# worldbench/lidarcrafter

Hardware: AMD Instinct MI355X
Metric: denoising-steps/sec, nuScenes 32×1024 range image, 1/2/4/8 GPU (higher is better)
Workload: dtype f16x2-split MFMA, fp32 accumulate (fp32-class accuracy)

## Files before the change

lidarcrafter_amd/csrc/conv_f16x2.hip:

```cpp
#include "conv_f16x2_common.h"

using namespace lcconv;

namespace {

#if LC_TIMING
__device__ unsigned long long lc_dbg[32];
#endif

#ifndef LC_NP_AUX
#define LC_NP_AUX LC_DEF_AUX
#endif
template <class C, bool WIDE = false, bool EMIT = false>
__global__ __launch_bounds__(256, (C::BN > 64 && C::NTAP == 9) ? 1 : 2) void conv_f16x2_kernel(ConvArgsH a) {
    constexpr int HALO = C::HALO, NTAP = C::NTAP, BN = C::BN;
    constexpr int XR = C::XR, XW = C::XW;
    constexpr int KS = 2 * HALO + 1;
    constexpr int CB = (NTAP == 1 && WIDE) ? ((BN <= 64 && C::TH_ * C::TW_ <= 128) ? 8 : 4) : C::CB;
    constexpr int XU = CB * XR * XW, NXU = (XU + 255) / 256;
    constexpr int WU = NTAP * CB * BN, NWU = (WU + 255) / 256;
    __shared__ half8 lds[2 * XU + 2 * WU];
    __shared__ f32x4 ctab[GN_MAX_C];
    __shared__ float2 gtab[GN_MAX_G];
    half8* xh = lds;
// ... 330 lines not shown
                        : OOB_W;
    }
    const unsigned w_chunk = (unsigned)CB * (unsigned)a.Cop * 16u;
    auto dma_w = [&](half8* buf, int q, int ch) {
        if (!(LC_ABLATE & 2)) lds_dma16(rs_w, (lds_vptr)(buf + loff_w[q]), voff_w[q], (unsigned)ch * w_chunk);
    };

    auto load_x = [&](float (&xr)[NXU][8], int ch) {
#pragma unroll
        for (int i = 0; i < NXU; ++i)
#pragma unroll
            for (int k = 0; k < 8; ++k)
                xr[i][k] = __builtin_bit_cast(
                    float, __builtin_amdgcn_raw_buffer_load_b32(rsrc, x_voff[i],
                                                                (unsigned)(ch * 16 + k) * HW * 4u, 0));
    };

    for (int i = tid; i < BN; i += NT)
        bias_s[i] = (a.bias && co0 + i < a.Co) ? a.bias[co0 + i] * (1.0f / out_unscale) : 0.0f;
    const int kh = lane >> 5, l31 = lane & 31;
    f32x16 acc[C::TCO_][C::TPX_];
    auto acc_init = [&]() {
#pragma unroll
        for (int i = 0; i < C::TCO_; ++i)
#pragma unroll
            for (int m = 0; m < 4; ++m) {
                const f32x4 bq = *reinterpret_cast<const f32x4*>(&bias_s[(wco * C::TCO_ + i) * 32 + 8 * m + 4 * kh]);
#pragma unroll
                for (int j = 0; j < C::TPX_; ++j) {
                    acc[i][j][4 * m] = bq.x; acc[i][j][4 * m + 1] = bq.y;
                    acc[i][j][4 * m + 2] = bq.z; acc[i][j][4 * m + 3] = bq.w;
                }
            }
    };

    int xbase[C::TPX_];
#pragma unroll
    for (int j = 0; j < C::TPX_; ++j) {
        const int t = wpx * C::TPX_ + j;
        const int tr = t / C::TPR, tc = t - tr * C::TPR;
        xbase[j] = kh * (XR * XW) + tr * XW + tc * 32 + l31;
    }
    const int wbase = kh * BN + wco * C::TCO_ * 32 + l31;

    const float silu_c = -1.4426950408889634f * a.range->x_unscale;
    half8 st_hi[NXU], st_lo[NXU];
    auto read_row = [&](int i, int q, int ch) -> f32x4 {
        if constexpr (GNM != 0) {
            const f32x4* g = x_ok[i] ? ctab + ch * 8 + x_cb[i] * 4 : ctab + (a.Cgn >> 1);
            return g[q];
        } else {
            return f32x4{0.f, 0.f, 0.f, 0.f};
        }
    };
    auto stage_pair = [&](float (&xr)[NXU][8], int i, int q, const f32x4 row) {
        if (LC_ABLATE & 1) { asm volatile("" ::"v"(xr[i][2 * q]), "v"(xr[i][2 * q + 1])); return; }
        half2v ph, pl;
        if constexpr (GNM != 0) {
            f32x2 v = {xr[i][2 * q], xr[i][2 * q + 1]};
            const f32x2 A = {row.x, row.y}, Bv = {row.z, row.w};
            v = __builtin_elementwise_fma(v, A, Bv);
            if constexpr (GNM == 1) {
                const f32x2 t = v * silu_c;
                f32x2 e = {__builtin_amdgcn_exp2f(t.x), __builtin_amdgcn_exp2f(t.y)};
                e = e + 1.0f;
                const f32x2 rc = {__builtin_amdgcn_rcpf(e.x), __builtin_amdgcn_rcpf(e.y)};
                v = v * rc;
            }
            pair_split_amax(v.x, v.y, ph, pl, am);
        } else {
            pair_split_scale<false>(xr[i][2 * q], xr[i][2 * q + 1], xs, ph, pl, am);
        }
        st_hi[i][2 * q] = ph.x; st_hi[i][2 * q + 1] = ph.y;
        st_lo[i][2 * q] = pl.x; st_lo[i][2 * q + 1] = pl.y;
    };
    auto commit_x = [&](half8* buf, int i) {
        if (LC_ABLATE & 1) return;
        const int d = x_rc[i] >= 0 ? x_cb[i] * PL + ((x_rc[i] >> 16) & 0xFFF) * XW + (x_rc[i] & 0xFFFF) : XU;
        buf[d] = st_hi[i];
        buf[XUP + d] = st_lo[i];
    };
    constexpr int NSTEP = 4 * NXU;
    constexpr int SPT = NTAP == 1 ? NSTEP : ((NSTEP + NTAP - 2) / (NTAP - 1) > 2 ? (NSTEP + NTAP - 2) / (NTAP - 1) : 2);
    auto step_tap = [](int st) {
        if (NTAP == 1) return 0;
        const int ntaps = (NSTEP + SPT - 1) / SPT;
        const int first = NTAP - 1 - ntaps > 0 ? NTAP - 1 - ntaps : 0;
        return first + st / SPT;
    };
    typedef DefEpi<C, EMIT_STATS> DE;
    DE de;
    auto compute = [&](const half8* cur, half8* nxt, float (&xr)[NXU][8], int chn, int dslot0) {
        const half8* cxh = cur;
        const half8* cxl = cur + XUP;
        const half8* cwh = cur + 2 * XUP;
        const half8* cwl = cwh + WS;
        half8 ah[2][C::TCO_], al[2][C::TCO_], bh[2][C::TPX_], bl[2][C::TPX_];
        auto fetch = [&](int tap, int s) {
            const int dy = tap / KS, dx = tap - dy * KS;
#pragma unroll
            for (int i = 0; i < C::TCO_; ++i) {
                ah[s][i] = cwh[tap * CB * BN + wbase + i * 32];
                al[s][i] = cwl[tap * CB * BN + wbase + i * 32];
            }
#pragma unroll
            for (int j = 0; j < C::TPX_; ++j) {
                bh[s][j] = cxh[xbase[j] + dy * XW + dx];
                bl[s][j] = cxl[xbase[j] + dy * XW + dx];
            }
        };
        fetch(0, 0);
#if LC_DMA_FIRST
        if (NTAP != 1) {
#pragma unroll
            for (int q = 0; q < KW; ++q) dma_w(nxt, q, chn);
        }
#endif
#pragma unroll
        for (int tap = 0; tap < NTAP; ++tap) {
            const int s = (LC_ABLATE & 4) ? 0 : (tap & 1);
            f32x4 rows[SPT];
            if (LC_PIPE_ROWS && GNM != 0) {
#pragma unroll
                for (int st = 0; st < NSTEP; ++st)
                    if (tap == step_tap(st)) rows[st % SPT] = read_row(st >> 2, st & 3, chn);
                __builtin_amdgcn_sched_barrier(0);
            }
            if (tap + 1 < NTAP && !(LC_ABLATE & 4)) fetch(tap + 1, s ^ 1);
            __builtin_amdgcn_sched_barrier(0);
            if (dslot0 >= 0 && dslot0 + tap < DE::NUSED) de.slot(dslot0 + tap);
            if (NTAP == 1) {
#pragma unroll
                for (int q = 0; q < KW; ++q) dma_w(nxt, q, chn);
            } else if (tap < KW && !LC_DMA_FIRST) {
                dma_w(nxt, tap, chn);
            }
#pragma unroll
            for (int st = 0; st < NSTEP; ++st)
                if (tap == step_tap(st)) {
                    stage_pair(xr, st >> 2, st & 3,
                               (LC_PIPE_ROWS && GNM != 0) ? rows[st % SPT] : read_row(st >> 2, st & 3, chn));
                    if ((st & 3) == 3) commit_x(nxt, st >> 2);
                }
            if (LC_ABLATE & 32) {
#pragma unroll
                for (int i = 0; i < C::TCO_; ++i) asm volatile("" ::"v"(ah[s][i]), "v"(al[s][i]));
#pragma unroll
                for (int j = 0; j < C::TPX_; ++j) asm volatile("" ::"v"(bh[s][j]), "v"(bl[s][j]));
                __builtin_amdgcn_sched_barrier(0);
                continue;
            }
            if (LC_F16X2_TERMS & 2) {
#pragma unroll
                for (int i = 0; i < C::TCO_; ++i)
#pragma unroll
                    for (int j = 0; j < C::TPX_; ++j)
                        acc[i][j] = __builtin_amdgcn_mfma_f32_32x32x16_f16(al[s][i], bh[s][j], acc[i][j], 0, 0, 0);
            }
            if (LC_F16X2_TERMS & 4) {
#pragma unroll
                for (int i = 0; i < C::TCO_; ++i)
#pragma unroll
                    for (int j = 0; j < C::TPX_; ++j)
                        acc[i][j] = __builtin_amdgcn_mfma_f32_32x32x16_f16(ah[s][i], bl[s][j], acc[i][j], 0, 0, 0);
            }
#pragma unroll
            for (int i = 0; i < C::TCO_; ++i)
#pragma unroll
                for (int j = 0; j < C::TPX_; ++j)
                    acc[i][j] = __builtin_amdgcn_mfma_f32_32x32x16_f16(ah[s][i], bh[s][j], acc[i][j], 0, 0, 0);
            __builtin_amdgcn_sched_barrier(0);
        }
    };

    half8* cur = lds;
    half8* nxt = lds + BUF;
    const int nchunk = a.Cib / CB;
    const int last = nchunk - 1;
    float xr[NXU][8];
    load_x(xr, 0);
#pragma unroll
    for (int q = 0; q < KW; ++q) dma_w(cur, q, 0);
    if constexpr (GNM != 0) {
        if (a.gs.partials) {
            for (int i = tid; i < a.Cgn; i += NT) ctab[i] = gn_row_from_stats(a.gs, xb, b, i, a.Ci, HW);
        } else if (a.segs.seg[0].p) {
            gn_rows_from_ostats<NT>(a, b, tid, ctab, gtab);
        } else {
            const f32x4* g = a.gn + (long long)b * a.Cgn;
            for (int i = tid; i < a.Cgn; i += NT) ctab[i] = g[i];
        }
        __syncthreads();
        constexpr int NQ = (GN_MAX_C / 2 + NT - 1) / NT;
        const int npair = a.Cgn >> 1;
        f32x4 qd[NQ];
#pragma unroll
        for (int k = 0; k < NQ; ++k) {
            const int p = tid + k * NT;
            if (p < npair) {
                const f32x4 r0 = ctab[2 * p], r1 = ctab[2 * p + 1];
                qd[k] = f32x4{r0.y * xs, r1.y * xs, fmaf(-r0.x, r0.y, r0.z) * xs, fmaf(-r1.x, r1.y, r1.z) * xs};
            }
        }
        __syncthreads();
#pragma unroll
        for (int k = 0; k < NQ; ++k) {
            const int p = tid + k * NT;
            if (p < npair) ctab[p] = qd[k];
        }
        if (tid < 4) ctab[npair + tid] = f32x4{0.f, 0.f, 0.f, 0.f};
        __syncthreads();
    }
#pragma unroll
    for (int i = 0; i < NXU; ++i) {
#pragma unroll
        for (int q = 0; q < 4; ++q) stage_pair(xr, i, q, read_row(i, q, 0));
        commit_x(cur, i);
    }
    asm volatile("s_waitcnt vmcnt(0)" ::: "memory");
    __syncthreads();
    const int co_wave = co0 + wco * C::TCO_ * 32 + 4 * kh;
    float* yb = a.y + (long long)b * a.y_bs;
    const float* rb = (a.res && !(LC_ABLATE & 16)) ? a.res + (long long)b * a.res_bs : nullptr;
    de.init(yb, rb, a.Co, HW, out_unscale, a.out_scale, co_wave,
            a.ostats ? a.ostats + (long long)b * (a.Co >> (a.ounit == 2 ? 1 : 3)) * a.oslots : nullptr, a.oslots,
            a.ounit);
    acc_init();
#if LC_TIMING
    unsigned long long t_comp = 0, t_bar = 0, t_epi = 0, n_chunk = 0;
    const unsigned long long t_start = __builtin_amdgcn_s_memtime();
#endif
    auto k_iter = [&](int nxt_ch, int dslot0) {
        if (!(LC_ABLATE & 2)) load_x(xr, nxt_ch);
        __builtin_amdgcn_sched_barrier(0);
#if LC_TIMING
        const unsigned long long ta = __builtin_amdgcn_s_memtime();
#endif
        compute(cur, nxt, xr, nxt_ch, dslot0);
#if LC_TIMING
        const unsigned long long tb = __builtin_amdgcn_s_memtime();
#endif
        {
            int later = 0;
#pragma unroll
            for (int tap = (NTAP == 1 ? 1 : (LC_DMA_FIRST ? 0 : KW)); tap < NTAP; ++tap) {
                const int sl = dslot0 + tap;
                if (dslot0 >= 0 && sl < DE::NUSED) later += DE::ops_of(sl);
            }
            wait_vmcnt(later);
        }
        asm volatile("s_waitcnt lgkmcnt(0)" ::: "memory");
        __builtin_amdgcn_s_barrier();
        asm volatile("" ::: "memory");
#if LC_TIMING
        t_comp += tb - ta; t_bar += __builtin_amdgcn_s_memtime() - tb; ++n_chunk;
#endif
        half8* t = cur; cur = nxt; nxt = t;
    };
    for (int tile = 0; tile < tpb; ++tile) {
        const bool more = tile + 1 < tpb;
        auto iter = [&](int ch, int dslot0) {
            if (ch == last && more) set_tile(h0 + dh, w0 + dw);
            k_iter(ch == last ? (more ? 0 : last) : ch + 1, dslot0);
        };
#pragma unroll
        for (int c = 0; c < DE::DCH; ++c)
            if (c < nchunk) iter(c, c * NTAP);
        if (nchunk < DE::DCH) {
            if (nchunk == 1) de.flush_from(NTAP);
            else if (nchunk == 2) de.flush_from(2 * NTAP);
            else de.flush_from(3 * NTAP);
        }
        for (int ch = DE::DCH; ch < nchunk; ++ch) iter(ch, -1);
        de.begin(acc, h0, w0, H, W, wpx, lane, a.tiles_w, HW, co0 + wco * C::TCO_ * 32, more);
        if (more) acc_init();
        h0 += dh; w0 += dw;
    }
#if LC_TIMING
    const unsigned long long te0 = __builtin_amdgcn_s_memtime();
#endif
    de.drain(acc);
#if LC_TIMING
    t_epi = __builtin_amdgcn_s_memtime() - te0;
#endif
    publish_amax(a.range, am, amax_seen);
#if LC_TIMING
    if (lane == 0) {
        atomicAdd(&lc_dbg[0], __builtin_amdgcn_s_memtime() - t_start);
        atomicAdd(&lc_dbg[1], t_start - t_enter);
        atomicAdd(&lc_dbg[2], t_comp);
        atomicAdd(&lc_dbg[3], t_bar);
        atomicAdd(&lc_dbg[4], t_epi);
        atomicAdd(&lc_dbg[5], n_chunk);
        atomicAdd(&lc_dbg[6], 1ull);
    }
#endif
}


#include "conv_f16x2_pp.h"

#include "conv_f16x2_ps.h"

template <class C>
int launch_pipe(ConvArgsH a, hipStream_t st) {
    a.tiles_h = (a.H + C::TH_ - 1) / C::TH_;
    a.tiles_w = (a.W + C::TW_ - 1) / C::TW_;
    const int ncot = (a.Co + C::BN - 1) / C::BN;
    const long long n_tiles = (long long)a.B * a.tiles_h * a.tiles_w * ncot;
    auto max_tpb = [&](int extent) {
        int t = 1;
        while (t < 4 && extent % (t * 2) == 0 && n_tiles / (t * 2) >= 256) t *= 2;
        return t;
    };
    static const int vert_env = [] { const char* e = getenv("LC_CONV_VERT"); return e ? atoi(e) : 1; }();
    static const int xcd_env = [] { const char* e = getenv("LC_CONV_XCD"); return e ? atoi(e) : 1; }();
    const int tpb_h = max_tpb(a.tiles_h), tpb_w = max_tpb(a.tiles_w);
    int vert = vert_env && tpb_h >= tpb_w;
    int tpb = vert ? tpb_h : tpb_w;
    if (C::NTAP == 1) tpb = 1;
    if (a.tpb > 0) {
        tpb = a.tpb;
        vert = vert_env && a.tiles_h % tpb == 0;
        if (!vert && a.tiles_w % tpb) tpb = 1;
    }
    if (a.part) tpb = 1;
    a.tpb = tpb;
    a.vert = vert;
    dim3 grid(a.B * a.tiles_h * a.tiles_w / tpb, ncot);
    a.xcd = (xcd_env && grid.x % 8 == 0 && grid.x >= 16) ? 1 : 0;

    if (a.xsp) {
        if constexpr (C::NTAP == 9) {
            if (a.part) grid.z = a.ksplit;
            if (a.ostats && !a.part) hipLaunchKernelGGL((conv_f16x2_ps_kernel<C, true>), grid, dim3(C::NT), 0, st, a);
            else hipLaunchKernelGGL((conv_f16x2_ps_kernel<C, false>), grid, dim3(C::NT), 0, st, a);
            return lc_launch_status();
        } else {
            return LC_EUNSUP;
        }
    }
    {
        const long long d = (const char*)a.wl - (const char*)a.wh;
        if (d <= 0 || d >= (1ll << 31)) return LC_EINVAL;
        if (d + (long long)C::NTAP * a.Cib * a.Cop * 16 >= (1ll << 31)) return LC_EUNSUP;
    }
    const int gnm = a.gn ? (a.gn_silu ? 1 : 2) : 0;
#define LC_PIPE_LAUNCH(E, G) hipLaunchKernelGGL((conv_f16x2_pipe_kernel<C, E, G>), grid, dim3(C::NT), 0, st, a)
    if (a.ostats && a.ounit == 2) {
        if constexpr (C::NTAP == 9) {
            if (gnm == 1) LC_PIPE_LAUNCH(2, 1); else if (gnm == 2) LC_PIPE_LAUNCH(2, 2); else LC_PIPE_LAUNCH(2, 0);
        } else {
            return LC_EUNSUP;
        }
    } else if (a.ostats) {
        if (gnm == 1) LC_PIPE_LAUNCH(1, 1); else if (gnm == 2) LC_PIPE_LAUNCH(1, 2); else LC_PIPE_LAUNCH(1, 0);
    } else {
        if (gnm == 1) LC_PIPE_LAUNCH(0, 1); else if (gnm == 2) LC_PIPE_LAUNCH(0, 2); else LC_PIPE_LAUNCH(0, 0);
    }
#undef LC_PIPE_LAUNCH
    return lc_launch_status();
}

template <class C>
int launch_h(ConvArgsH a, hipStream_t st) {
    a.tiles_h = (a.H + C::TH_ - 1) / C::TH_;
    a.tiles_w = (a.W + C::TW_ - 1) / C::TW_;
    dim3 grid(a.B * a.tiles_h * a.tiles_w, (a.Co + C::BN - 1) / C::BN);
    if constexpr (C::NTAP == 1) {
        const bool wide = (long long)grid.x * grid.y <= 512;
        if (a.ostats) {
            if (a.ounit != 8) return LC_EUNSUP;
            if (wide) hipLaunchKernelGGL((conv_f16x2_kernel<C, true, true>), grid, dim3(256), 0, st, a);
            else hipLaunchKernelGGL((conv_f16x2_kernel<C, false, true>), grid, dim3(256), 0, st, a);
            return lc_launch_status();
        }
        if (wide) {
            hipLaunchKernelGGL((conv_f16x2_kernel<C, true>), grid, dim3(256), 0, st, a);
            return lc_launch_status();
        }
    } else if (a.ostats) {
        return LC_EUNSUP;
    }
    hipLaunchKernelGGL((conv_f16x2_kernel<C, false>), grid, dim3(256), 0, st, a);
    return lc_launch_status();
}

bool pp_eligible(int Ci, int Co, int H, int W, int ks) {
    return ks == 3 && Ci % 16 == 0 && Ci >= 64 && Ci <= PPG::MAX_C && Co % 64 == 0 && H % 4 == 0 && W % 64 == 0;
}
int launch_pp(ConvArgsH a, hipStream_t st) {
    if (!pp_eligible(a.Ci, a.Co, a.H, a.W, 3) || a.xsp || a.part) return LC_EUNSUP;
    if (a.gn && a.Cgn > PPG::MAX_C) return LC_EUNSUP;
    a.tiles_h = a.H / PPG::TH;
    a.tiles_w = a.W / PPG::TW;
    const int ncot = a.Co / PPG::BN;
    const long long strips = (long long)a.B * a.tiles_h * a.tiles_w * ncot;
    int ns = 1;
    while (ns < 8 && a.tiles_h % (2 * ns) == 0 && strips / (2 * ns) >= 256) ns *= 2;
    if (a.tpb > 0 && a.tiles_h % a.tpb == 0) ns = a.tpb;
    a.tpb = ns;
    dim3 grid(a.B * a.tiles_h * a.tiles_w / ns, ncot);
    static const int xcd_env = [] { const char* e = getenv("LC_CONV_XCD"); return e ? atoi(e) : 1; }();
    a.xcd = (xcd_env && grid.x % 8 == 0 && grid.x >= 16) ? 1 : 0;
    a.vert = 1;
    {
        const long long d = (const char*)a.wl - (const char*)a.wh;
        if (d <= 0 || d >= (1ll << 31)) return LC_EINVAL;
        if (d + (long long)PPG::NTAP * a.Cib * a.Cop * 16 >= (1ll << 31)) return LC_EUNSUP;
    }
    const int gnm = a.gn ? (a.gn_silu ? 1 : 2) : 0;
#define LC_PP_LAUNCH(E, G) hipLaunchKernelGGL((conv_f16x2_pp_kernel<E, G>), grid, dim3(PPG::NT), 0, st, a)
    if (a.ostats && a.ounit == 2) {
        if (gnm == 1) LC_PP_LAUNCH(2, 1); else if (gnm == 2) LC_PP_LAUNCH(2, 2); else LC_PP_LAUNCH(2, 0);
    } else if (a.ostats) {
        if (gnm == 1) LC_PP_LAUNCH(1, 1); else if (gnm == 2) LC_PP_LAUNCH(1, 2); else LC_PP_LAUNCH(1, 0);
    } else {
        if (gnm == 1) LC_PP_LAUNCH(0, 1); else if (gnm == 2) LC_PP_LAUNCH(0, 2); else LC_PP_LAUNCH(0, 0);
    }
#undef LC_PP_LAUNCH
    return lc_launch_status();
}

template <int KS>
int dispatch_h(int cfg, const ConvArgsH& a, hipStream_t st) {
    switch (cfg) {
        case 1: return launch_h<HCfg<2, 2, 2, 2, 2, 64, KS>>(a, st);
        case 2: return launch_h<HCfg<1, 4, 2, 2, 4, 64, KS>>(a, st);
        case 3: return launch_h<HCfg<2, 2, 1, 1, 2, 32, KS>>(a, st);
        case 4: return launch_h<HCfg<2, 2, 2, 2, 4, 32, KS>>(a, st);
        case 5: return launch_h<HCfg<1, 4, 2, 1, 2, 64, KS>>(a, st);
        case 12: return launch_pipe<HCfg<1, 4, 2, 2, 4, 64, KS>>(a, st);
        case 13: return launch_pipe<HCfg<2, 2, 1, 1, 2, 32, KS>>(a, st);
        case 15: return launch_pipe<HCfg<1, 4, 2, 1, 2, 64, KS>>(a, st);
        case 22: return launch_pipe<HCfg<1, 8, 2, 1, 4, 64, KS>>(a, st);
        case 23: return launch_pipe<HCfg<2, 4, 1, 2, 4, 64, KS>>(a, st);
        case 25: return launch_pipe<HCfg<2, 4, 1, 1, 2, 64, KS>>(a, st);
        case 27:
            if (KS == 3 && tall_eligible(a)) return launch_tall(a, st);
            return launch_pipe<HCfg<2, 4, 1, 2, 4, 64, KS>>(a, st);
        case 28: return launch_pipe<HCfg<1, 8, 1, 1, 4, 64, KS>>(a, st);
        case 33: return KS == 3 ? launch_pp(a, st) : LC_EUNSUP;
        default: return LC_EUNSUP;
    }
}

int pipe_stat_slots(int cfg, int H, int W, int ks = 3) {
    int th, tw, wpx;
    switch (cfg) {
        case 1: if (ks != 1) return 0; th = 2; tw = 64; wpx = 2; break;
        case 2: if (ks != 1) return 0; th = 4; tw = 64; wpx = 4; break;
        case 3: if (ks != 1) return 0; th = 2; tw = 32; wpx = 2; break;
        case 4: if (ks != 1) return 0; th = 4; tw = 32; wpx = 2; break;
        case 5: if (ks != 1) return 0; th = 2; tw = 64; wpx = 4; break;
        case 12: th = 4; tw = 64; wpx = 4; break;
        case 13: th = 2; tw = 32; wpx = 2; break;
        case 15: th = 2; tw = 64; wpx = 4; break;
        case 22: th = 4; tw = 64; wpx = 8; break;
        case 23: th = 4; tw = 64; wpx = 4; break;
        case 25: th = 2; tw = 64; wpx = 4; break;
        case 27: th = 4; tw = 64; wpx = 4; break;
        case 28: th = 4; tw = 64; wpx = 8; break;
        case 33: th = 4; tw = 64; wpx = 4; break;
        default: return 0;
    }
    return ((H + th - 1) / th) * ((W + tw - 1) / tw) * wpx;
}

int auto_cfg_h(int B, int Ci, int Co, int H, int W, int ks) {
    const long long px = (long long)B * H * W;
    auto blocks = [&](int bn, int pxb) { return ((Co + bn - 1) / bn) * ((px + pxb - 1) / pxb); };
    const bool t256 = H % 4 == 0 && W % 64 == 0, t128 = H % 2 == 0 && W % 64 == 0;
    if (ks == 1) {
        if (t256 && blocks(64, 256) > 192 && blocks(64, 256) <= 256) return 23;
        return (t128 && blocks(64, 128) >= 512) ? 5 : 3;
    }
    if (Ci >= 24) {
        if (Co <= 32 && t256 && blocks(64, 256) >= 256) return 28;
        static const long long pp_min = [] { const char* e = getenv("LC_PP_MIN_STRIPS"); return e ? atoll(e) : 0ll; }();
        if (pp_min > 0 && pp_eligible(Ci, Co, H, W, ks) && blocks(64, 256) >= pp_min) return 33;
        if (t256 && blocks(64, 256) >= 256) {
            static const int tall_env = [] { const char* e = getenv("LC_TALL"); return e ? atoi(e) : 1; }();
            if (tall_env && ks == 3 && (Ci == 32 || Ci == 64)) return 27;
            return 23;
        }
        if (t128 && blocks(64, 128) >= 256) return 25;
        return 13;
    }
    if (t256 && blocks(64, 256) >= 256 && Ci >= 64) return 2;
    if (t128 && blocks(64, 128) >= 512) return 5;
    return 3;
}

__global__ void weight_amax_kernel(const float* __restrict__ w, long long n, float* wmeta) {
    float am = 0.0f;
    for (long long e = blockIdx.x * (long long)blockDim.x + threadIdx.x; e < n;
         e += (long long)gridDim.x * blockDim.x)
        am = fmaxf(am, fabsf(w[e]));
    lc_block_amax_publish(am, reinterpret_cast<unsigned*>(wmeta + 2));
}

__device__ __forceinline__ float weight_scale_for(float amax) {
    if (!(amax > 0.0f) || !(amax < 3.0e38f)) return W_PRESCALE_DEFAULT;
    const float A = amax * W_PRESCALE_DEFAULT;
    if (A >= 32.0f && A <= 32768.0f) return W_PRESCALE_DEFAULT;
    int e;
    frexpf(amax, &e);
    int k = 13 - e;
    k = k < -120 ? -120 : (k > 120 ? 120 : k);
    return ldexpf(1.0f, k);
}

template <bool DX>
__device__ __forceinline__ void pack_weight_elems(const float* __restrict__ w, _Float16* __restrict__ ph,
                                                  _Float16* __restrict__ pl, int Co, int Ci, int ntap, int Cib,
                                                  int Cop, float ws, long long first, long long stride) {
    const long long n = (long long)ntap * Cib * Cop * 8;
    for (long long e = first; e < n; e += stride) {
        const int k = e & 7;
        long long r = e >> 3;
        const int co = r % Cop; r /= Cop;
        const int cb = r % Cib;
        const int tap = r / Cib;
        const int ci = cb * 8 + k;
        float v = 0.0f;
        if (co < Co && ci < Ci)
            v = (DX ? w[((long long)ci * Co + co) * ntap + (ntap - 1 - tap)]
                    : w[((long long)co * Ci + ci) * ntap + tap]) * ws;
        _Float16 hf, lf;
        f16x2_split_scalar(v, hf, lf);
        ph[e] = hf;
        pl[e] = lf;
    }
}

template <bool DX>
__global__ void pack_weight_h_kernel(const float* __restrict__ w, _Float16* __restrict__ ph,
                                     _Float16* __restrict__ pl, int Co, int Ci, int ntap, int Cib,
                                     int Cop, float* wmeta, const float* __restrict__ amax_src) {
    const float amax = amax_src ? amax_src[2] : wmeta[2];
    const float ws = weight_scale_for(amax);
    if (blockIdx.x == 0 && threadIdx.x == 0) {
        wmeta[0] = ws; wmeta[1] = 1.0f / ws;
        if (amax_src) { wmeta[2] = amax; wmeta[3] = 0.0f; }
    }
    pack_weight_elems<DX>(w, ph, pl, Co, Ci, ntap, Cib, Cop, ws, blockIdx.x * (long long)blockDim.x + threadIdx.x,
                          (long long)gridDim.x * blockDim.x);
}

__global__ void multi_weight_zero_kernel(const lc_weight_pack_job* __restrict__ jobs, int n) {
    const int j = blockIdx.x * blockDim.x + threadIdx.x;
    if (j < n) jobs[j].fwd_meta[2] = 0.0f;
}
__global__ void multi_weight_amax_kernel(const lc_weight_pack_job* __restrict__ jobs) {
    const lc_weight_pack_job jb = jobs[blockIdx.y];
    const long long n = (long long)jb.Co * jb.Ci * jb.ks * jb.ks;
    float am = 0.0f;
    for (long long e = blockIdx.x * (long long)blockDim.x + threadIdx.x; e < n; e += (long long)gridDim.x * blockDim.x)
        am = fmaxf(am, fabsf(jb.w[e]));
    lc_block_amax_publish(am, reinterpret_cast<unsigned*>(jb.fwd_meta + 2));
}
__global__ void multi_weight_pack_kernel(const lc_weight_pack_job* __restrict__ jobs) {
    const lc_weight_pack_job jb = jobs[blockIdx.y];
    const float amax = jb.fwd_meta[2];
    const float ws = weight_scale_for(amax);
    const int ntap = jb.ks * jb.ks;
    const long long first = blockIdx.x * (long long)blockDim.x + threadIdx.x, stride = (long long)gridDim.x * blockDim.x;
    if (blockIdx.z == 0) {
        if (blockIdx.x == 0 && threadIdx.x == 0) { jb.fwd_meta[0] = ws; jb.fwd_meta[1] = 1.0f / ws; }
        pack_weight_elems<false>(jb.w, (_Float16*)jb.fwd_hi, (_Float16*)jb.fwd_lo, jb.Co, jb.Ci, ntap,
                                 (jb.Ci + 15) / 16 * 2, (jb.Co + 63) / 64 * 64, ws, first, stride);
    } else {
        if (blockIdx.x == 0 && threadIdx.x == 0) {
            jb.dx_meta[0] = ws; jb.dx_meta[1] = 1.0f / ws; jb.dx_meta[2] = amax; jb.dx_meta[3] = 0.0f;
        }
        pack_weight_elems<true>(jb.w, (_Float16*)jb.dx_hi, (_Float16*)jb.dx_lo, jb.Ci, jb.Co, ntap,
                                (jb.Co + 15) / 16 * 2, (jb.Ci + 63) / 64 * 64, ws, first, stride);
    }
}

}

extern "C" int64_t lc_packed_conv_weight_f16x2_elems(int Co, int Ci, int ks) {
    const int64_t Cip = (Ci + 15) / 16 * 16, Cop = (Co + 63) / 64 * 64;
    return (int64_t)ks * ks * Cip * Cop;
}

namespace {
int pack_weight_h(const float* w, void* wp_hi, void* wp_lo, int Co, int Ci, int ks, float* wmeta,
                  const float* amax_src, bool dx, lc_stream_t s) {
    if (!w || !wp_hi || !wp_lo || !wmeta || Co <= 0 || Ci <= 0 || (ks != 1 && ks != 3)) return LC_EINVAL;
    const int Cib = (Ci + 15) / 16 * 2, Cop = (Co + 63) / 64 * 64;
    const long long n = (long long)ks * ks * Cib * Cop * 8;
    const long long nw = (long long)Co * Ci * ks * ks;
    const int blocks = (int)((n + 255) / 256 > 4096 ? 4096 : (n + 255) / 256);
    const int ablocks = (int)((nw + 255) / 256 > 1024 ? 1024 : (nw + 255) / 256);
    if (!amax_src) {
        if (hipMemsetAsync(wmeta, 0, 4 * sizeof(float), lc_s(s)) != hipSuccess) return lc_launch_status();
        hipLaunchKernelGGL(weight_amax_kernel, dim3(ablocks), dim3(256), 0, lc_s(s), w, nw, wmeta);
    }
    if (dx)
        hipLaunchKernelGGL(pack_weight_h_kernel<true>, dim3(blocks), dim3(256), 0, lc_s(s), w, (_Float16*)wp_hi,
                           (_Float16*)wp_lo, Co, Ci, ks * ks, Cib, Cop, wmeta, amax_src);
    else
        hipLaunchKernelGGL(pack_weight_h_kernel<false>, dim3(blocks), dim3(256), 0, lc_s(s), w, (_Float16*)wp_hi,
                           (_Float16*)wp_lo, Co, Ci, ks * ks, Cib, Cop, wmeta, amax_src);
    return lc_launch_status();
}
}

extern "C" int lc_pack_conv_weight_f16x2(const float* w, void* wp_hi, void* wp_lo, int Co, int Ci,
                                         int ks, float* wmeta, lc_stream_t s) {
    return pack_weight_h(w, wp_hi, wp_lo, Co, Ci, ks, wmeta, nullptr, false, s);
}

extern "C" int lc_pack_conv_weights_f16x2_multi(const lc_weight_pack_job* jobs, int n, int with_dx, lc_stream_t s) {
    if (!jobs || n <= 0) return LC_EINVAL;
    hipLaunchKernelGGL(multi_weight_zero_kernel, dim3((n + 255) / 256), dim3(256), 0, lc_s(s), jobs, n);
    hipLaunchKernelGGL(multi_weight_amax_kernel, dim3(16, n), dim3(256), 0, lc_s(s), jobs);
    hipLaunchKernelGGL(multi_weight_pack_kernel, dim3(48, n, with_dx ? 2 : 1), dim3(256), 0, lc_s(s), jobs);
    return lc_launch_status();
}

extern "C" int lc_pack_conv_weight_f16x2_dx(const float* w_fwd, void* wp_hi, void* wp_lo, int Co, int Ci, int ks,
                                            float* wmeta, const float* wmeta_fwd, lc_stream_t s) {
    return pack_weight_h(w_fwd, wp_hi, wp_lo, Co, Ci, ks, wmeta, wmeta_fwd, true, s);
}

__global__ void tensor_amax_kernel(const float* __restrict__ x, long long x_bs, long long n, int B,
                                   lc_conv_range* rg) {
    float am = 0.0f;
    const long long n4 = n >> 2;
    for (int b = blockIdx.y; b < B; b += gridDim.y) {
        const float* p = x + b * x_bs;
        if ((reinterpret_cast<unsigned long long>(p) & 15) == 0) {
            const f32x4* p4 = reinterpret_cast<const f32x4*>(p);
            for (long long e = blockIdx.x * (long long)blockDim.x + threadIdx.x; e < n4;
                 e += (long long)gridDim.x * blockDim.x) {
                const f32x4 v = p4[e];
                am = fmaxf(fmaxf(am, fmaxf(fabsf(v.x), fabsf(v.y))), fmaxf(fabsf(v.z), fabsf(v.w)));
            }
            for (long long e = (n4 << 2) + blockIdx.x * (long long)blockDim.x + threadIdx.x; e < n;
                 e += (long long)gridDim.x * blockDim.x)
                am = fmaxf(am, fabsf(p[e]));
        } else {
            for (long long e = blockIdx.x * (long long)blockDim.x + threadIdx.x; e < n;
                 e += (long long)gridDim.x * blockDim.x)
                am = fmaxf(am, fabsf(p[e]));
        }
    }
    lc_block_amax_publish(am, reinterpret_cast<unsigned*>(&rg->reserved));
}
__device__ __forceinline__ void range_record_set(lc_conv_range* rg, float amax) {
    float sc = X_PRESCALE_DEFAULT;
    if (amax > 0.0f && amax < 3.0e38f) {
        int e;
        frexpf(amax, &e);
        int k = 13 - e;
        k = k < -120 ? -120 : (k > 120 ? 120 : k);
        sc = ldexpf(1.0f, k);
    }
    rg->x_scale = sc;
    rg->x_unscale = 1.0f / sc;
    rg->amax_scaled = 0.0f;
    rg->reserved = 0.0f;
}
__global__ void range_set_kernel(lc_conv_range* rg) { range_record_set(rg, rg->reserved); }
__global__ void range_from_amax_kernel(lc_conv_range* rg, const float* __restrict__ amax, long long n, float bound_mult) {
    float m = 0.0f;
    for (long long i = threadIdx.x; i < n; i += blockDim.x) m = fmaxf(m, amax[i]);
#pragma unroll
    for (int o = 32; o > 0; o >>= 1) m = fmaxf(m, __shfl_xor(m, o, 64));
    __shared__ float wm[4];
    if ((threadIdx.x & 63) == 0) wm[threadIdx.x >> 6] = m;
    __syncthreads();
    if (threadIdx.x == 0) range_record_set(rg, fmaxf(fmaxf(wm[0], wm[1]), fmaxf(wm[2], wm[3])) * bound_mult);
}

extern "C" int lc_range_from_tensor(const float* x, int64_t x_bs, int B, int64_t n, lc_conv_range* range,
                                    lc_stream_t s) {
    if (!x || !range || B <= 0 || n <= 0) return LC_EINVAL;
    long long bx = (n / 4 + 255) / 256;
    bx = bx < 1 ? 1 : (bx > 512 ? 512 : bx);
    const int by = B < 8 ? B : 8;
    hipLaunchKernelGGL(tensor_amax_kernel, dim3((unsigned)bx, by), dim3(256), 0, lc_s(s), x, (long long)x_bs,
                       (long long)n, B, range);
    hipLaunchKernelGGL(range_set_kernel, dim3(1), dim3(1), 0, lc_s(s), range);
    return lc_launch_status();
}

extern "C" int lc_range_from_amax(const float* amax, int64_t n, float bound_mult, lc_conv_range* range, lc_stream_t s) {
    if (!amax || n <= 0 || !range || !(bound_mult >= 1.0f)) return LC_EINVAL;
    hipLaunchKernelGGL(range_from_amax_kernel, dim3(1), dim3(256), 0, lc_s(s), range, amax, (long long)n, bound_mult);
    return lc_launch_status();
}

extern "C" int lc_conv2d_ring_f16x2_fwd(const float* x, int64_t x_bs, const void* wp_hi,
                                        const void* wp_lo, const float* bias, const float* res,
                                        int64_t res_bs, float* y, int64_t y_bs, int B, int Ci,
                                        int Co, int H, int W, int ks, float out_scale, int tile_cfg,
                                        const float* gn_coeffs, int gn_cpad, int gn_silu,
                                        const lc_gn_stats_input* gn_stats, float* gn_ostats_out, int gn_ostats_unit,
                                        const float* wmeta, lc_conv_range* range, lc_stream_t s) {
    if (!x || !wp_hi || !wp_lo || !y || !wmeta || !range || B <= 0 || Ci <= 0 || Co <= 0 || H <= 0 ||
        W <= 0)
        return LC_EINVAL;
    if (ks != 1 && ks != 3) return LC_EUNSUP;
    if ((long long)H * W >= (1 << 24)) return LC_EUNSUP;
    if ((long long)Ci * H * W * 4 >= (1ll << 31) || (long long)Co * H * W * 4 >= (1ll << 31)) return LC_EUNSUP;
    ConvArgsH a;
    a.x = x; a.wh = (const half8*)wp_hi; a.wl = (const half8*)wp_lo; a.bias = bias; a.res = res;
    a.y = y; a.x_bs = x_bs; a.res_bs = res_bs; a.y_bs = y_bs;
    a.range = range; a.wmeta = wmeta;
    a.xsp = nullptr; a.xsp_bs = 0; a.xsp_c8 = 0; a.part = nullptr; a.ksplit = 0;
    a.B = B; a.Ci = Ci; a.Co = Co; a.H = H; a.W = W;
    a.Cib = (Ci + 15) / 16 * 2; a.Cop = (Co + 63) / 64 * 64;
    a.out_scale = out_scale;
    a.tiles_h = a.tiles_w = 0;
    a.gn = reinterpret_cast<const f32x4*>(gn_coeffs);
    a.Cgn = gn_cpad; a.gn_silu = gn_silu;
    a.gs = lc_gn_stats_input{nullptr, 0, 0, 0.f, nullptr, nullptr, nullptr, nullptr, 0, nullptr, nullptr};
    a.segs = STAT_SEGS_NONE;
    if (gn_stats) {
        if (gn_coeffs || gn_stats->G <= 0 || Ci % gn_stats->G) return LC_EINVAL;
        if (gn_stats->partials) {
            if (gn_stats->nch <= 0) return LC_EINVAL;
        } else {
            if (const int rc = stat_segs_from(gn_stats->os0, gn_stats->os1, Ci, Ci / gn_stats->G, LC_EINVAL, a.segs)) return rc;
            if (gn_stats->G > GN_MAX_G) return LC_EUNSUP;
        }
        a.gs = *gn_stats;
        a.gs.os0 = a.gs.os1 = nullptr;
        a.gn = reinterpret_cast<const f32x4*>(x);
        a.Cgn = gn_cpad > 0 ? gn_cpad : (Ci + 15) / 16 * 16;
    }
    a.tpb = 0;
    if (tile_cfg >= 100) { a.tpb = tile_cfg / 100; tile_cfg %= 100; }
    if (a.gn && (a.Cgn < (Ci + 15) / 16 * 16 || a.Cgn > GN_MAX_C || (a.Cgn & 1))) return LC_EINVAL;
    if (ks == 1 && ((long long)H * W) % 128 == 0) {
        a.H = H = (int)(((long long)H * W) / 64);
        a.W = W = 64;
    }
    if (tile_cfg == 0) tile_cfg = auto_cfg_h(B, Ci, Co, H, W, ks);
    a.ostats = nullptr; a.oslots = 0; a.ounit = 8;
    if (gn_ostats_out) {
        if (gn_ostats_unit != 8 && gn_ostats_unit != 2) return LC_EINVAL;
        a.oslots = pipe_stat_slots(tile_cfg, H, W, ks);
        if (a.oslots <= 0 || Co % 8) return LC_EUNSUP;
        a.ostats = reinterpret_cast<f32x4*>(gn_ostats_out);
        a.ounit = gn_ostats_unit;
    }
    return ks == 3 ? dispatch_h<3>(tile_cfg, a, lc_s(s)) : dispatch_h<1>(tile_cfg, a, lc_s(s));
}

#if LC_TIMING
extern "C" int lc_debug_read(unsigned long long* out16, int reset) {
    hipDeviceSynchronize();
    hipMemcpyFromSymbol(out16, HIP_SYMBOL(lc_dbg), sizeof(unsigned long long) * 32);
    if (reset) { unsigned long long z[32] = {0}; hipMemcpyToSymbol(HIP_SYMBOL(lc_dbg), z, sizeof(z)); }
    return 0;
}
#endif

extern "C" int64_t lc_conv2d_ring_f16x2_stats_slots(int B, int Ci, int Co, int H, int W, int ks,
                                                    int tile_cfg) {
    if (B <= 0 || Ci <= 0 || Co <= 0 || Co % 8 || H <= 0 || W <= 0 || (ks != 1 && ks != 3)) return 0;
    if (tile_cfg >= 100) tile_cfg %= 100;
    if (ks == 1 && ((long long)H * W) % 128 == 0) { H = (int)(((long long)H * W) / 64); W = 64; }
    if (tile_cfg == 0) tile_cfg = auto_cfg_h(B, Ci, Co, H, W, ks);
    return pipe_stat_slots(tile_cfg, H, W, ks);
}

extern "C" int lc_conv2d_ring_f16x2_ps_fwd(const void* x_split, const void* wp_hi, const void* wp_lo,
                                           const float* bias, const float* res, int64_t res_bs,
                                           float* y, int64_t y_bs, int B, int Ci, int Co, int H, int W,
                                           float out_scale, int tile_cfg, float* gn_ostats_out, int gn_ostats_unit,
                                           float* splitk_part, int ksplit, const float* wmeta,
                                           lc_conv_range* range, lc_stream_t s) {
    if (!x_split || !wp_hi || !wp_lo || (!y && !splitk_part) || !wmeta || !range || B <= 0 || Ci <= 0 ||
        Co <= 0 || H <= 0 || W <= 0)
        return LC_EINVAL;
    if (Ci % 16) return LC_EUNSUP;
    if (splitk_part && (ksplit < 2 || ksplit > Ci / 16)) return LC_EINVAL;
    if ((long long)H * W >= (1 << 24) || (long long)2 * (Ci / 8) * H * W * 16 >= (1ll << 31)) return LC_EUNSUP;
    if ((long long)Co * H * W * 4 >= (1ll << 31)) return LC_EUNSUP;
    ConvArgsH a;
    a.x = nullptr; a.wh = (const half8*)wp_hi; a.wl = (const half8*)wp_lo; a.bias = bias; a.res = res;
    a.y = y; a.x_bs = 0; a.res_bs = res_bs; a.y_bs = y_bs;
    a.range = range; a.wmeta = wmeta;
    a.B = B; a.Ci = Ci; a.Co = Co; a.H = H; a.W = W;
    a.Cib = Ci / 8; a.Cop = (Co + 63) / 64 * 64;
    if (a.wl != a.wh + (long long)9 * a.Cib * a.Cop) return LC_EINVAL;
    a.xsp = (const half8*)x_split; a.xsp_c8 = Ci / 8; a.xsp_bs = (long long)2 * (Ci / 8) * H * W;
    a.part = splitk_part; a.ksplit = splitk_part ? ksplit : 0;
    a.out_scale = out_scale;
    a.tiles_h = a.tiles_w = 0;
    a.gn = nullptr; a.Cgn = 0; a.gn_silu = 0;
    a.gs = lc_gn_stats_input{nullptr, 0, 0, 0.f, nullptr, nullptr, nullptr, nullptr, 0, nullptr, nullptr};
    a.segs = STAT_SEGS_NONE;
    a.tpb = 0;
    if (tile_cfg >= 100) { a.tpb = tile_cfg / 100; tile_cfg %= 100; }
    if (tile_cfg == 0) tile_cfg = auto_cfg_h(B, Ci < 24 ? 24 : Ci, Co, H, W, 3);
    if (pipe_stat_slots(tile_cfg, H, W) <= 0) return LC_EUNSUP;
    a.ostats = nullptr; a.oslots = 0; a.ounit = 8;
    if (gn_ostats_out && !splitk_part) {
        a.oslots = pipe_stat_slots(tile_cfg, H, W);
        if (Co % 8 || (gn_ostats_unit != 8 && gn_ostats_unit != 4)) return LC_EUNSUP;
        a.ostats = reinterpret_cast<f32x4*>(gn_ostats_out);
        a.ounit = gn_ostats_unit;
    }
    return dispatch_h<3>(tile_cfg, a, lc_s(s));
}

#include "conv_f16x2_ps1.h"

namespace {
__global__ __launch_bounds__(256) void splitk_reduce_kernel(const float* __restrict__ part, int ks,
                                                           const float* __restrict__ bias,
                                                           const float* __restrict__ res,
                                                           long long res_bs, float* __restrict__ y,
                                                           long long y_bs, int B, int Co, int HW,
                                                           float out_scale, f32x4* __restrict__ ostats,
                                                           int oslots) {
    const int b = blockIdx.z, oct = blockIdx.y, c0 = oct * 8;
    const int p = blockIdx.x * 256 + threadIdx.x;
    const bool pok = p < HW;
    const long long plane = (long long)B * Co * HW;
    float v[8];
    bool ok[8];
    const float* pp[8];
#pragma unroll
    for (int k = 0; k < 8; ++k) {
        ok[k] = pok && c0 + k < Co;
        pp[k] = part + ((long long)b * Co + (ok[k] ? c0 + k : c0)) * HW + (pok ? p : 0);
        v[k] = 0.0f;
    }
    int z = 0;
    for (; z + 1 < ks; z += 2) {
        float t0[8], t1[8];
#pragma unroll
        for (int k = 0; k < 8; ++k) { t0[k] = pp[k][z * plane]; t1[k] = pp[k][(z + 1) * plane]; }
#pragma unroll
        for (int k = 0; k < 8; ++k) v[k] = (v[k] + t0[k]) + t1[k];
    }
    if (z < ks) {
#pragma unroll
        for (int k = 0; k < 8; ++k) v[k] += pp[k][z * plane];
    }
    float bv[8], rv[8];
#pragma unroll
    for (int k = 0; k < 8; ++k) {
        bv[k] = (bias && ok[k]) ? bias[c0 + k] : 0.0f;
        rv[k] = (res && ok[k]) ? res[b * res_bs + (long long)(c0 + k) * HW + p] : 0.0f;
    }
#pragma unroll
    for (int k = 0; k < 8; ++k) {
        v[k] = ok[k] ? ((v[k] + bv[k]) + rv[k]) * out_scale : 0.0f;
        if (ok[k]) y[b * y_bs + (long long)(c0 + k) * HW + p] = v[k];
    }
    if (ostats) {
        StatAcc<PIVOT_FIRST> st;
        st.start(v[0]);
#pragma unroll
        for (int k = 0; k < 8; ++k) st.add(v[k], pok);
        const int nvalid = __popcll(__ballot(pok));
        const float s_ = wave_sum_to_lane63(st.s), q_ = wave_sum_to_lane63(st.q);
        const int slot = blockIdx.x * 4 + (threadIdx.x >> 6);
        if ((threadIdx.x & 63) == 63 && slot < oslots)
            ostats[((long long)b * (Co >> 3) + oct) * oslots + slot] =
                f32x4{st.p, (float)(8 * nvalid), s_, q_};
    }
}
}

extern "C" int64_t lc_splitk_stats_slots(int H, int W) {
    return H > 0 && W > 0 ? ((int64_t)H * W + 255) / 256 * 4 : 0;
}

extern "C" int lc_splitk_reduce(const float* part, int ksplit, const float* bias, const float* res,
                                int64_t res_bs, float* y, int64_t y_bs, int B, int Co, int H, int W,
                                float out_scale, float* gn_ostats_out, lc_stream_t s) {
    if (!part || !y || ksplit < 1 || B <= 0 || Co <= 0 || H <= 0 || W <= 0) return LC_EINVAL;
    if (gn_ostats_out && Co % 8) return LC_EUNSUP;
    const int HW = H * W;
    hipLaunchKernelGGL(splitk_reduce_kernel, dim3((HW + 255) / 256, (Co + 7) / 8, B), dim3(256), 0,
                       lc_s(s), part, ksplit, bias, res, (long long)res_bs, y, (long long)y_bs, B, Co, HW,
                       out_scale, reinterpret_cast<f32x4*>(gn_ostats_out),
                       (int)lc_splitk_stats_slots(H, W));
    return lc_launch_status();
}

LC_TOUCH_TU(conv_f16x2, tensor_amax_kernel)
```

Before: 280.8.

## Add intra-block split-K 1x1 conv kernel for small-spatial high-channel layers

Adds a new 1x1 convolution kernel that gives each block a small 64x64 (or 128x32) output tile and splits the input-channel reduction across its four waves. Each wave streams weights and activations straight from global memory into registers through a three-deep software prefetch, then the partial sums are reduced through LDS in the epilogue, which also applies bias, residual and GroupNorm statistics. The auto-selector routes 1x1 layers with Ci>=256 and few output tiles to this kernel, aiming to fill the GPU on low-resolution bottleneck layers where the existing tiling launches too few blocks. The cost is an extra LDS reduction and barrier per block plus no LDS reuse of operands. A timing script is included.

Result: no change. 283.0, median of 6 (+0.8%).

```diff
diff --git a/devtools/tok1x1_time.py b/devtools/tok1x1_time.py
--- /dev/null
+++ b/devtools/tok1x1_time.py
@@ -0,0 +1,51 @@
+import os
+import sys
+import time
+
+sys.path.insert(0, os.path.dirname(os.path.dirname(os.path.abspath(__file__))))
+import torch
+
+from lidarcrafter_amd import ops as K
+
+
+def arg(name, default):
+    return int(sys.argv[sys.argv.index(name) + 1]) if name in sys.argv else default
+
+
+B, ROUNDS, N = arg("--batch", 8), arg("--rounds", 5), 20
+SHAPES = [("out_proj d_block4", 512, 512, 4, 128, True, 0.5 ** 0.5, True),
+          ("skip u_block4", 512, 256, 4, 128, False, 1.0, False),
+          ("out_proj u_block4", 256, 256, 4, 128, True, 1.0, False),
+          ("skip u_block3", 512, 128, 8, 256, False, 1.0, False)]
+ROUTES = (3, 41, 42)
+dev = torch.device("cuda:0")
+print(f"batch {B}, {ROUNDS} rounds of {N} graph-replayed launches; us per launch: best / worst")
+for name, Ci, Co, H, W, use_res, scale, emit in SHAPES:
+    x = torch.randn(B, Ci, H, W, device=dev)
+    w = torch.randn(Co, Ci, 1, 1, device=dev) / Ci ** 0.5
+    b = torch.randn(Co, device=dev)
+    res = torch.randn(B, Co, H, W, device=dev) if use_res else None
+    out = torch.empty(B, Co, H, W, device=dev)
+    graphs = {}
+    for cfg in ROUTES:
+        pk = K.PackedConv()
+        f = lambda: K.conv2d_ring(x, pk, w, b, res=res, out=out, out_scale=scale, precision="f16x2", emit_stats=emit,
+                                  tile_cfg=cfg)
+        for _ in range(3):
+            f()
+        g = torch.cuda.CUDAGraph()
+        with torch.cuda.graph(g):
+            for _ in range(N):
+                f()
+        g.replay()
+        graphs[cfg] = g
+    torch.cuda.synchronize()
+    ts = {cfg: [] for cfg in graphs}
+    for _ in range(ROUNDS):
+        for cfg, g in graphs.items():
+            t0 = time.perf_counter()
+            g.replay()
+            torch.cuda.synchronize()
+            ts[cfg].append((time.perf_counter() - t0) / N * 1e6)
+    cols = "   ".join(f"cfg {cfg}: {min(v):6.1f} / {max(v):6.1f}" for cfg, v in ts.items())
+    print(f"{name:18s} {Ci:4d}->{Co:4d} @{B}x{H}x{W}: {cols}", flush=True)
diff --git a/lidarcrafter_amd/csrc/conv_f16x2.hip b/lidarcrafter_amd/csrc/conv_f16x2.hip
--- a/lidarcrafter_amd/csrc/conv_f16x2.hip
+++ b/lidarcrafter_amd/csrc/conv_f16x2.hip
@@ -656,6 +656,8 @@
 
 #include "conv_f16x2_ps.h"
 
+#include "conv_f16x2_tok.h"
+
 template <class C>
 int launch_pipe(ConvArgsH a, hipStream_t st) {
     a.tiles_h = (a.H + C::TH_ - 1) / C::TH_;
@@ -795,6 +797,8 @@
             return launch_pipe<HCfg<2, 4, 1, 2, 4, 64, KS>>(a, st);
         case 28: return launch_pipe<HCfg<1, 8, 1, 1, 4, 64, KS>>(a, st);
         case 33: return KS == 3 ? launch_pp(a, st) : LC_EUNSUP;
+        case TOK_CFG_2X2: return KS == 1 ? launch_tok<2, 2>(a, st) : LC_EUNSUP;
+        case TOK_CFG_4X1: return KS == 1 ? launch_tok<4, 1>(a, st) : LC_EUNSUP;
         default: return LC_EUNSUP;
     }
 }
@@ -816,17 +820,22 @@
         case 27: th = 4; tw = 64; wpx = 4; break;
         case 28: th = 4; tw = 64; wpx = 8; break;
         case 33: th = 4; tw = 64; wpx = 4; break;
+        case TOK_CFG_2X2: case TOK_CFG_4X1: return ks == 1 ? tok_stat_slots(H, W) : 0;
         default: return 0;
     }
     return ((H + th - 1) / th) * ((W + tw - 1) / tw) * wpx;
 }
 
-int auto_cfg_h(int B, int Ci, int Co, int H, int W, int ks) {
+int auto_cfg_h(int B, int Ci, int Co, int H, int W, int ks, bool tok = true) {
     const long long px = (long long)B * H * W;
     auto blocks = [&](int bn, int pxb) { return ((Co + bn - 1) / bn) * ((px + pxb - 1) / pxb); };
     const bool t256 = H % 4 == 0 && W % 64 == 0, t128 = H % 2 == 0 && W % 64 == 0;
     if (ks == 1) {
         if (t256 && blocks(64, 256) > 192 && blocks(64, 256) <= 256) return 23;
+        static const int tok_env = [] { const char* e = getenv("LC_TOK1X1"); return e ? atoi(e) : 1; }();
+        if (tok && tok_env && Ci >= 256 && blocks(64, 64) <= 512 && tok_takes(Ci, Co, H, W, ks) &&
+            tok_stat_slots(H, W) == pipe_stat_slots(3, H, W, 1))
+            return blocks(64, 64) <= 256 ? TOK_CFG_4X1 : TOK_CFG_2X2;
         return (t128 && blocks(64, 128) >= 512) ? 5 : 3;
     }
     if (Ci >= 24) {
@@ -844,6 +853,11 @@
     if (t256 && blocks(64, 256) >= 256 && Ci >= 64) return 2;
     if (t128 && blocks(64, 128) >= 512) return 5;
     return 3;
+}
+
+int resolve_tok_cfg(int cfg, int B, int Ci, int Co, int H, int W, int ks, bool fused_gn) {
+    if (!is_tok_cfg(cfg) || (!fused_gn && tok_takes(Ci, Co, H, W, ks))) return cfg;
+    return auto_cfg_h(B, Ci, Co, H, W, ks, false);
 }
 
 __global__ void weight_amax_kernel(const float* __restrict__ w, long long n, float* wmeta) {
@@ -1096,6 +1110,9 @@
         a.W = W = 64;
     }
     if (tile_cfg == 0) tile_cfg = auto_cfg_h(B, Ci, Co, H, W, ks);
+    const int asked_cfg = tile_cfg;
+    tile_cfg = resolve_tok_cfg(tile_cfg, B, Ci, Co, H, W, ks, a.gn != nullptr);
+    if (gn_ostats_out && pipe_stat_slots(tile_cfg, H, W, ks) != pipe_stat_slots(asked_cfg, H, W, ks)) return LC_EUNSUP;
     a.ostats = nullptr; a.oslots = 0; a.ounit = 8;
     if (gn_ostats_out) {
         if (gn_ostats_unit != 8 && gn_ostats_unit != 2) return LC_EINVAL;
@@ -1122,6 +1139,7 @@
     if (tile_cfg >= 100) tile_cfg %= 100;
     if (ks == 1 && ((long long)H * W) % 128 == 0) { H = (int)(((long long)H * W) / 64); W = 64; }
     if (tile_cfg == 0) tile_cfg = auto_cfg_h(B, Ci, Co, H, W, ks);
+    tile_cfg = resolve_tok_cfg(tile_cfg, B, Ci, Co, H, W, ks, false);
     return pipe_stat_slots(tile_cfg, H, W, ks);
 }
 
diff --git a/lidarcrafter_amd/csrc/conv_f16x2_tok.h b/lidarcrafter_amd/csrc/conv_f16x2_tok.h
--- /dev/null
+++ b/lidarcrafter_amd/csrc/conv_f16x2_tok.h
@@ -0,0 +1,216 @@
+template <int TCO, int TPX, bool EMIT>
+__global__ __launch_bounds__(256, 2) void conv_f16x2_tok_kernel(ConvArgsH a) {
+    constexpr int NW = 4, NSUB = TCO * TPX, DEPTH = 3;
+    static_assert(NSUB == NW, "one 32 x 32 sub-tile per wave in the epilogue");
+    constexpr int COB = TCO * 32, PXB = TPX * 32;
+    constexpr unsigned OOB = 0x80000000u;
+    __shared__ f32x4 red[NW * NSUB * 4 * 64];
+
+    const int tid = threadIdx.x;
+    const int lane = tid & 63;
+    const int wave = __builtin_amdgcn_readfirstlane(tid >> 6);
+    const int kh = lane >> 5, l31 = lane & 31;
+    const int HW = a.H * a.W;
+    const unsigned HW4 = (unsigned)HW * 4u;
+    const int b = blockIdx.x / a.tiles_w;
+    const int p0 = (blockIdx.x - b * a.tiles_w) * PXB;
+    const int co0 = blockIdx.y * COB;
+
+    const float xs = a.range->x_scale;
+    const float amax_seen = a.range->amax_scaled;
+    const float out_unscale = a.range->x_unscale * a.wmeta[1];
+    float am = 0.0f;
+
+    const __amdgpu_buffer_rsrc_t rs_x = __builtin_amdgcn_make_buffer_rsrc(
+        (void*)(a.x + (long long)b * a.x_bs), 0, (unsigned)a.Ci * HW4, 0x00020000);
+    const unsigned wbytes = (unsigned)a.Cib * (unsigned)a.Cop * 16u;
+    const __amdgpu_buffer_rsrc_t rs_wh = __builtin_amdgcn_make_buffer_rsrc((void*)a.wh, 0, wbytes, 0x00020000);
+    const __amdgpu_buffer_rsrc_t rs_wl = __builtin_amdgcn_make_buffer_rsrc((void*)a.wl, 0, wbytes, 0x00020000);
+    unsigned woff[TCO], xoff[TPX];
+#pragma unroll
+    for (int i = 0; i < TCO; ++i) {
+        const int co = co0 + i * 32 + l31;
+        woff[i] = co < a.Cop ? (unsigned)(kh * a.Cop + co) * 16u : OOB;
+    }
+#pragma unroll
+    for (int j = 0; j < TPX; ++j) {
+        const int p = p0 + j * 32 + l31;
+        xoff[j] = p < HW ? (unsigned)(8 * kh * HW + p) * 4u : OOB;
+    }
+    const unsigned wstep = 2u * (unsigned)a.Cop * 16u;
+    const unsigned xstep = 16u * HW4;
+
+    lc_u32x4 fah[DEPTH][TCO], fal[DEPTH][TCO];
+    float fx[DEPTH][TPX][8];
+    auto load = [&](int s, int ks) {
+        const unsigned wk = (unsigned)ks * wstep, xk = (unsigned)ks * xstep;
+#pragma unroll
+        for (int i = 0; i < TCO; ++i) {
+            fah[s][i] = __builtin_amdgcn_raw_buffer_load_b128(rs_wh, woff[i] + wk, 0, 0);
+            fal[s][i] = __builtin_amdgcn_raw_buffer_load_b128(rs_wl, woff[i] + wk, 0, 0);
+        }
+#pragma unroll
+        for (int j = 0; j < TPX; ++j)
+#pragma unroll
+            for (int k = 0; k < 8; ++k)
+                fx[s][j][k] = __builtin_bit_cast(
+                    float, __builtin_amdgcn_raw_buffer_load_b32(rs_x, xoff[j] + xk + (unsigned)k * HW4, 0, 0));
+    };
+
+    f32x16 acc[TCO][TPX];
+#pragma unroll
+    for (int i = 0; i < TCO; ++i)
+#pragma unroll
+        for (int j = 0; j < TPX; ++j)
+#pragma unroll
+            for (int r = 0; r < 16; ++r) acc[i][j][r] = 0.0f;
+
+    auto compute = [&](int s) {
+        half8 bh[TPX], bl[TPX], ah[TCO], al[TCO];
+#pragma unroll
+        for (int j = 0; j < TPX; ++j) split8<true>(fx[s][j], xs, bh[j], bl[j], am);
+#pragma unroll
+        for (int i = 0; i < TCO; ++i) {
+            ah[i] = __builtin_bit_cast(half8, fah[s][i]);
+            al[i] = __builtin_bit_cast(half8, fal[s][i]);
+        }
+        if (LC_F16X2_TERMS & 2) {
+#pragma unroll
+            for (int i = 0; i < TCO; ++i)
+#pragma unroll
+                for (int j = 0; j < TPX; ++j)
+                    acc[i][j] = __builtin_amdgcn_mfma_f32_32x32x16_f16(al[i], bh[j], acc[i][j], 0, 0, 0);
+        }
+        if (LC_F16X2_TERMS & 4) {
+#pragma unroll
+            for (int i = 0; i < TCO; ++i)
+#pragma unroll
+                for (int j = 0; j < TPX; ++j)
+                    acc[i][j] = __builtin_amdgcn_mfma_f32_32x32x16_f16(ah[i], bl[j], acc[i][j], 0, 0, 0);
+        }
+#pragma unroll
+        for (int i = 0; i < TCO; ++i)
+#pragma unroll
+            for (int j = 0; j < TPX; ++j)
+                acc[i][j] = __builtin_amdgcn_mfma_f32_32x32x16_f16(ah[i], bh[j], acc[i][j], 0, 0, 0);
+    };
+
+    const int nk = a.Cib >> 1;
+    const int nmine = nk > wave ? (nk - wave + NW - 1) / NW : 0;
+#pragma unroll
+    for (int s = 0; s < DEPTH - 1; ++s) load(s, wave + s * NW);
+    for (int it = 0; it < nmine; it += DEPTH) {
+#pragma unroll
+        for (int s = 0; s < DEPTH; ++s) {
+            if (it + s >= nmine) break;
+            load((s + DEPTH - 1) % DEPTH, wave + (it + s + DEPTH - 1) * NW);
+            __builtin_amdgcn_sched_barrier(0);
+            compute(s);
+            __builtin_amdgcn_sched_barrier(0);
+        }
+    }
+    publish_amax(a.range, am, amax_seen);
+
+    const int oi = wave / TPX, oj = wave - oi * TPX;
+    const float* rb = a.res ? a.res + (long long)b * a.res_bs : nullptr;
+    const __amdgpu_buffer_rsrc_t rs_y = __builtin_amdgcn_make_buffer_rsrc((void*)(a.y + (long long)b * a.y_bs), 0,
+                                                                         (unsigned)a.Co * HW4, 0x00020000);
+    const __amdgpu_buffer_rsrc_t rs_r = __builtin_amdgcn_make_buffer_rsrc((void*)rb, 0, rb ? (unsigned)a.Co * HW4 : 0u,
+                                                                         0x00020000);
+    const __amdgpu_buffer_rsrc_t rs_b = __builtin_amdgcn_make_buffer_rsrc((void*)a.bias, 0,
+                                                                         a.bias ? (unsigned)a.Co * 4u : 0u, 0x00020000);
+    const int co_sub = co0 + oi * 32;
+    const int co_wave = co_sub + 4 * kh;
+    const int p = p0 + oj * 32 + l31;
+    const bool pok = p < HW;
+    const unsigned vo = pok ? (unsigned)(co_wave * HW + p) * 4u : OOB;
+    float bias_r[16], res_r[16];
+#pragma unroll
+    for (int r = 0; r < 16; ++r) {
+        const int cor = mfma_row(r);
+        const bool cok = co_wave + cor < a.Co;
+        bias_r[r] = __builtin_bit_cast(float, __builtin_amdgcn_raw_buffer_load_b32(
+                                                  rs_b, cok ? (unsigned)(co_wave + cor) * 4u : OOB, 0, 0));
+        res_r[r] = __builtin_bit_cast(float, __builtin_amdgcn_raw_buffer_load_b32(rs_r, cok ? vo : OOB, (unsigned)cor * HW4, 0));
+    }
+#pragma unroll
+    for (int i = 0; i < TCO; ++i)
+#pragma unroll
+        for (int j = 0; j < TPX; ++j)
+#pragma unroll
+            for (int m = 0; m < 4; ++m)
+                red[((wave * NSUB + i * TPX + j) * 4 + m) * 64 + lane] =
+                    f32x4{acc[i][j][4 * m], acc[i][j][4 * m + 1], acc[i][j][4 * m + 2], acc[i][j][4 * m + 3]};
+    __syncthreads();
+    float sum[16];
+#pragma unroll
+    for (int m = 0; m < 4; ++m) {
+        f32x4 t[NW];
+#pragma unroll
+        for (int w = 0; w < NW; ++w) t[w] = red[((w * NSUB + wave) * 4 + m) * 64 + lane];
+        f32x4 v = t[0];
+#pragma unroll
+        for (int w = 1; w < NW; ++w) v = v + t[w];
+        sum[4 * m] = v.x; sum[4 * m + 1] = v.y; sum[4 * m + 2] = v.z; sum[4 * m + 3] = v.w;
+    }
+
+    StatAcc<PIVOT_WAVE> st[4];
+#pragma unroll
+    for (int r = 0; r < 16; ++r) {
+        const int cor = mfma_row(r);
+        float v = sum[r] * out_unscale;
+        v += bias_r[r];
+        v += res_r[r];
+        v *= a.out_scale;
+        __builtin_amdgcn_raw_buffer_store_b32(__builtin_bit_cast(unsigned, v), rs_y, co_wave + cor < a.Co ? vo : OOB,
+                                              (unsigned)cor * HW4, LC_NP_AUX);
+        if constexpr (EMIT) {
+            const int m = r >> 2;
+            if ((r & 3) == 0) st[m].start(pok ? v : 0.0f);
+            st[m].add(v, pok);
+        }
+    }
+    if constexpr (EMIT) {
+        const int nvalid = __popcll(__ballot(pok) & 0xFFFFFFFFull);
+        const int slot = (p0 >> 5) + oj;
+        const __amdgpu_buffer_rsrc_t rs_o = __builtin_amdgcn_make_buffer_rsrc(
+            (void*)(a.ostats + (long long)b * (a.Co >> 3) * a.oslots), 0, (unsigned)(a.Co >> 3) * (unsigned)a.oslots * 16u,
+            0x00020000);
+        const float nv = (float)(8 * nvalid);
+#pragma unroll
+        for (int m = 0; m < 4; ++m) {
+            const int co_oct = co_sub + 8 * m;
+            const float sf = wave_sum_to_lane63(st[m].s), qf = wave_sum_to_lane63(st[m].q);
+            const unsigned eo = (lane >= 60 && co_oct < a.Co && slot < a.oslots)
+                                    ? ((unsigned)(co_oct >> 3) * (unsigned)a.oslots + (unsigned)slot) * 16u + 4u * (lane & 3)
+                                    : OOB;
+            store_entry_4lanes(rs_o, st[m].p, nv, sf, qf, eo);
+        }
+    }
+}
+
+constexpr int TOK_CFG_2X2 = 41, TOK_CFG_4X1 = 42;
+inline bool is_tok_cfg(int cfg) { return cfg == TOK_CFG_2X2 || cfg == TOK_CFG_4X1; }
+
+inline bool tok_takes(int Ci, int Co, int H, int W, int ks) {
+    const long long HW = (long long)H * W, Cib = (Ci + 15) / 16 * 2, Cop = (Co + 63) / 64 * 64;
+    return ks == 1 && (Cib * 8 + 256) * HW * 4 < (1ll << 31) && (Cib + 32) * Cop * 16 < (1ll << 31) &&
+           (long long)Co * HW * 4 < (1ll << 31);
+}
+inline int tok_stat_slots(int H, int W) { return (int)(((long long)H * W + 31) / 32); }
+
+template <int TCO, int TPX>
+int launch_tok(ConvArgsH a, hipStream_t st) {
+    if (a.gn || a.xsp || a.part || !tok_takes(a.Ci, a.Co, a.H, a.W, 1)) return LC_EUNSUP;
+    const int HW = a.H * a.W;
+    a.tiles_h = 1;
+    a.tiles_w = (HW + TPX * 32 - 1) / (TPX * 32);
+    const dim3 grid((unsigned)(a.B * a.tiles_w), (unsigned)((a.Co + TCO * 32 - 1) / (TCO * 32)));
+    if (a.ostats) {
+        if (a.ounit != 8 || a.oslots != tok_stat_slots(a.H, a.W)) return LC_EUNSUP;
+        hipLaunchKernelGGL((conv_f16x2_tok_kernel<TCO, TPX, true>), grid, dim3(256), 0, st, a);
+    } else {
+        hipLaunchKernelGGL((conv_f16x2_tok_kernel<TCO, TPX, false>), grid, dim3(256), 0, st, a);
+    }
+    return lc_launch_status();
+}
```
